# Matrixeigs/PowerSystemsReliabilityAssessment

Hardware: AMD Instinct MI355X
Metric: Monte Carlo DC-OPF scenarios/sec (RTS-24 HL2 non-sequential) (higher is better)
Workload: dtype f64

## Files before the change

### powersystemsreliabilityassessment_amd/csrc/relmc_core.hip

```cpp
#include <hip/hip_runtime.h>

#include <cmath>
#include <cstddef>
#include <cstdio>
#include <cstdlib>
#include <cstring>
#include <memory>
#include <new>
#include <type_traits>

#include "relmc_ctx.h"
#ifdef RELMC_DEV_SWITCHES
#include "relmc_dev_switches.h"
#endif
#include "relmc_kernels.hip"

static_assert(sizeof(relmc::DevAcc) == sizeof(relmc_acc), "device accumulator image must match relmc_acc");

namespace relmc_host {

const char* const kNoCtx = "relmc: null context";

int fail(relmc_ctx* ctx, int code, const std::string& msg)
{
// ... 9 lines not shown
    a.feastol = o.feastol; a.gradtol = o.gradtol; a.comptol = o.comptol; a.costtol = o.costtol;
    a.xi = o.xi; a.sigma = o.sigma; a.z0 = o.z0; a.alpha_min = o.alpha_min; a.max_stepsize = o.max_stepsize;
    a.fail_threshold = 1e-4;
    return a;
}

namespace {
template <class TL>
int grid_for(relmc_ctx* ctx, int64_t n)
{
    const int64_t groups = ((n + TL::SPW - 1) / TL::SPW + TL::WPB - 1) / TL::WPB;
    int64_t g = (int64_t)ctx->num_cu * ctx->blocks_per_cu;
    if (g > groups) g = groups;
    if (g < 1) g = 1;
    return (int)g;
}

template <int MODE, class TL>
int launch_eval_t(relmc_ctx* ctx, EvalArgs& a, int* rows_out, hipEvent_t ev_start, hipEvent_t ev_stop, int alt)
{
    int blocks = grid_for<TL>(ctx, a.n);
    if (MODE == 6) {
        if (blocks > 64) blocks = 64;
        const size_t n = 2 * (size_t)ctx->nb, stride = n * (n + 1), need = stride * (size_t)blocks * TL::WPB * TL::SPW;
        HIP_TRY(ctx, ctx->retry.dense.grow(need));
        a.dense = ctx->retry.dense.get(); a.dense_stride = stride;
    }
    HIP_TRY(ctx, ctx->dpartial.grow(sizeof(PartialT<TL>) * 64 * TL::WPB * (size_t)blocks));
    a.partial = ctx->dpartial.get();
    a.scen_doubles = alt ? ctx->alt_scen_doubles[alt - 1] : ctx->scen_doubles;
    a.prio_mode = blocks != ctx->num_cu * ctx->blocks_per_cu ? 0u : (ctx->blocks_per_cu == 2 ? 1u : (ctx->blocks_per_cu == 1 && TL::WPB >= 8 ? 2u : 0u));
    a.stash_off = alt ? ctx->alt_stash_off[alt - 1] : ctx->stash_off;
    a.case_bytes = (uint32_t)offsetof(DevCaseT<TL>, task);
#if defined(RELMC_PHASE_TIMING) || defined(RELMC_TRACE)
    HIP_TRY(ctx, ctx->dtiming.grow(8 * 65536));
    a.timing = ctx->dtiming.get(); ctx->timing_waves = blocks * TL::WPB;
#else
    a.timing = nullptr;
#endif
    a.tail_groups = 0;
    if constexpr (MODE == 0 && std::is_same<TL, Tile24>::value) {
        a.tail_rec = nullptr; a.tail_count = nullptr;
        const TailPlan plan(a.n, (int64_t)blocks * TL::WPB);
        if (plan.T > 0 && !ctx->sw.static_tail) {
            { const int rc = fail_count_ensure(ctx); if (rc) return rc; }
            HIP_TRY(ctx, ctx->dtail.grow(sizeof(TailRecT<TL>) * (size_t)plan.items()));
            a.tail_groups = plan.T; a.tail_rec = ctx->dtail.get(); a.tail_count = ctx->retry.fail_count.get() + 1;
        }
        ctx->last_tail_groups = a.tail_groups; ctx->tail_launches += a.tail_groups > 0;
        if (verbose()) fprintf(stderr, "relmc: fused launch of %lld scenarios on %d wavefronts: tail groups T = %d%s\n", (long long)a.n, blocks * TL::WPB, a.tail_groups,
                               a.tail_groups ? "" : (ctx->sw.static_tail ? " (static_tail)" : " (fewer than 2 T groups per wavefront)"));
    }
    HIP_TRY(ctx, hipEventRecord(ev_start ? ev_start : ctx->ev0, ctx->stream));
    bool launched = false;
    if constexpr (MODE == 0 && std::is_same<TL, Tile24>::value) {
        if (alt == 0 && ctx->shape_static && !ctx->sw.dynamic_shape) {
            hipLaunchKernelGGL((relmc_eval_kernel<0, Tile24, ShapeRts24>), dim3(blocks), dim3(64 * Tile24::WPB), ctx->lds_bytes, ctx->stream,
                               reinterpret_cast<const DevCaseT<Tile24>*>(ctx->dcase.get()), a);
            launched = true;
        }
    }
    if (!launched)
        hipLaunchKernelGGL((relmc_eval_kernel<MODE, TL>), dim3(blocks), dim3(64 * TL::WPB), alt ? ctx->alt_lds_bytes[alt - 1] : ctx->lds_bytes, ctx->stream,
                           reinterpret_cast<const DevCaseT<TL>*>(alt ? ctx->dcase_alt[alt - 1].get() : ctx->dcase.get()), a);
    HIP_TRY(ctx, hipGetLastError());
    if constexpr (MODE == 0 && std::is_same<TL, Tile24>::value) {
// ... 417 lines not shown
```

### powersystemsreliabilityassessment_amd/csrc/relmc_ctx.h

```cpp
#pragma once
#include <hip/hip_runtime.h>

#include <cmath>
#include <cstdint>
#include <functional>
#include <memory>
#include <string>
#include <type_traits>
#include <vector>

#include "../../include/relmc.h"
#include "relmc_dev.h"

struct relmc_switches {
    bool no_retry = false;
    bool retry_dense_first = false;
    bool nsq_no_stretch = false;
    bool db_no_probe = false;
    bool dynamic_shape = false;
    bool static_tail = false;
};

namespace relmc_host {
template <class T, bool Pinned = false>
class Buffer {
public:
    Buffer() = default;
    Buffer(Buffer&& o) noexcept : p_(o.p_), n_(o.n_) { o.p_ = nullptr; o.n_ = 0; }
    Buffer& operator=(Buffer&& o) noexcept
    {
        if (this != &o) { reset(); p_ = o.p_; n_ = o.n_; o.p_ = nullptr; o.n_ = 0; }
        return *this;
    }
    ~Buffer() { reset(); }
    T* get() const { return p_; }
    size_t size() const { return n_; }
    void reset()
    {
        if (p_) (void)(Pinned ? hipHostFree(p_) : hipFree(p_));
        p_ = nullptr; n_ = 0;
    }
    hipError_t grow(size_t n)
    {
        if (n <= n_) return hipSuccess;
        reset();
        void* p = nullptr;
        const hipError_t e = Pinned ? hipHostMalloc(&p, sizeof(T) * n, hipHostMallocDefault) : hipMalloc(&p, sizeof(T) * n);
        if (e == hipSuccess) { p_ = static_cast<T*>(p); n_ = n; }
        return e;
    }
private:
    T* p_ = nullptr;
    size_t n_ = 0;
// ... 298 lines not shown
```

### powersystemsreliabilityassessment_amd/csrc/relmc_debug.hip

```cpp
#include <cstdio>
#include <cstring>
#include <memory>

#include "relmc_ctx.h"
#include "relmc_shape_rts24.h"

using namespace relmc_host;

extern "C" {

int32_t relmc_debug_schedule(const relmc_ctx* ctx, int32_t* out9)
{
    if (!ctx || !out9 || !ctx->has_case) return RELMC_ERR_INVALID;
    auto fill = [&](const auto& C) {
        int ntask = 0;
        for (int p = 0; p < C.npass; ++p) ntask += C.pass_ntask[p];
        out9[0] = C.npass_upd; out9[1] = C.npass_inv; out9[2] = C.npass - C.npass_upd - C.npass_inv; out9[3] = C.noff;
        out9[4] = C.nzero; out9[5] = (int)C.nws; out9[6] = (int)ctx->lds_bytes; out9[7] = ctx->blocks_per_cu; out9[8] = ntask;
        if (verbose()) fprintf(stderr, "relmc: modelled LDS conflict cycles per Newton step %ld -> %ld\n", ctx->conflict_before, ctx->conflict_after);
        if (verbose()) fprintf(stderr, "relmc: longest line / injection list per bus slot: %d %d / %d %d\n", (int)C.maxdeg_s[0], (int)C.maxdeg_s[1], (int)C.maxinj_s[0], (int)C.maxinj_s[1]);
        if (verbose()) { fprintf(stderr, "relmc: tasks per pass:"); for (int p = 0; p < C.npass; ++p) fprintf(stderr, " %d", (int)C.pass_ntask[p]); fprintf(stderr, "\n"); }
    };
    if (ctx->tile == 0) fill(ctx->hcase24); else fill(ctx->hcase96);
    return RELMC_OK;
// ... 10 lines not shown
    std::vector<uint32_t> keys((size_t)n * ow, 0u);
    for (int64_t r = 0; r < n; ++r) for (int k = 0; k < ncomp; ++k) if (states_host[(size_t)r * ncomp + k]) keys[(size_t)r * ow + (k >> 5)] |= 1u << (k & 31);
    DevBuf<uint32_t> dk; DevBuf<double> dd, dn; DevBuf<int32_t> dm;
    if (dk.grow(keys.size()) != hipSuccess || dd.grow((size_t)n) != hipSuccess || dm.grow((size_t)n) != hipSuccess || dn.grow((size_t)n * nb) != hipSuccess)
        return fail(ctx, RELMC_ERR_HIP, "dense simulation: device allocation failed");
    int rc = RELMC_OK;
    if (hipMemcpy(dk.get(), keys.data(), sizeof(uint32_t) * keys.size(), hipMemcpyHostToDevice) != hipSuccess) rc = fail(ctx, RELMC_ERR_HIP, "dense simulation: H2D failed");
    EvalArgs a = make_args(o);
    a.n = n; a.memo_keys = dk.get(); a.db_first = 0; a.dns = dd.get(); a.status = dm.get(); a.nodal = dn.get();
    int rows = 0;
    if (rc == RELMC_OK) rc = launch_eval(ctx, 6, a, &rows);
    if (rc == RELMC_OK) rc = finish_timing(ctx);
    std::vector<int32_t> meta((size_t)n);
    if (rc == RELMC_OK && (hipMemcpy(dns_host, dd.get(), sizeof(double) * (size_t)n, hipMemcpyDeviceToHost) != hipSuccess ||
                           hipMemcpy(meta.data(), dm.get(), sizeof(int32_t) * (size_t)n, hipMemcpyDeviceToHost) != hipSuccess ||
                           (nodal_host && hipMemcpy(nodal_host, dn.get(), sizeof(double) * (size_t)n * nb, hipMemcpyDeviceToHost) != hipSuccess)))
        rc = fail(ctx, RELMC_ERR_HIP, "dense simulation: D2H failed");
    if (rc) return rc;
    for (int64_t r = 0; r < n; ++r) { if (status_host) status_host[r] = meta[(size_t)r] & 3; if (iters_host) iters_host[r] = (int32_t)((uint32_t)meta[(size_t)r] >> 8); }
    return RELMC_OK;
}

int32_t relmc_debug_phase_cycles(relmc_ctx* ctx, unsigned long long* out8)
{
    if (!ctx || !out8) return RELMC_ERR_INVALID;
    for (int k = 0; k < 8; ++k) out8[k] = 0;
    if (!ctx->dtiming.get() || ctx->timing_waves <= 0) return RELMC_OK;
    std::vector<unsigned long long> h((size_t)ctx->timing_waves * 8);
    HIP_TRY(ctx, hipMemcpy(h.data(), ctx->dtiming.get(), h.size() * sizeof(unsigned long long), hipMemcpyDeviceToHost));
    for (int w = 0; w < ctx->timing_waves; ++w) for (int k = 0; k < 8; ++k) out8[k] += h[(size_t)w * 8 + k];
    return RELMC_OK;
}

int32_t relmc_debug_trace(relmc_ctx* ctx, double* out, int32_t n_doubles)
{
    if (!ctx || !out || n_doubles < 0) return RELMC_ERR_INVALID;
    for (int k = 0; k < n_doubles; ++k) out[k] = 0.0;
    if (!ctx->dtiming.get() || n_doubles > 8 * 65536) return RELMC_OK;
    HIP_TRY(ctx, hipMemcpy(out, ctx->dtiming.get(), sizeof(double) * n_doubles, hipMemcpyDeviceToHost));
    return RELMC_OK;
}

int32_t relmc_debug_shape(const relmc_case_desc* d, const int32_t* order_hint, int32_t n_hint, int32_t* case_out, int32_t* static_out)
{
    if (static_out) ShapeRts24::values(static_out);
    if (case_out) {
        if (!d) return RELMC_ERR_INVALID;
        SymOpts so = sym_opts_default();
        if (order_hint && n_hint > 0) { so.order_hint = order_hint; so.n_hint = n_hint; }
        std::string err;
        SymGeom g;
        const int rc = with_symbolic(d, 0, so, g, err, [&](const auto& C) { shape_of(C, g.stash_off, g.scen_doubles, case_out); return (int)RELMC_OK; });
        if (rc) return rc < 0 ? rc : -rc;
    }
    return SF_COUNT;
}

int64_t relmc_debug_stretch_len(int64_t batch, int64_t done, double beta, double beta_limit, int64_t round, int32_t* final_out)
{
    if (batch <= 0 || batch > kStretchMaxBatch || done < 0 || round < 0) return RELMC_ERR_INVALID;
    const Stretch s = stretch_length(batch, done, beta, beta_limit, stretch_per(batch), round);
    if (final_out) *final_out = s.final ? 1 : 0;
    return s.len;
}

int32_t relmc_debug_shape_path(const relmc_ctx* ctx)
{
    if (!ctx || !ctx->has_case) return RELMC_ERR_INVALID;
    return ctx->shape_static && !ctx->sw.dynamic_shape ? 1 : 0;
}

int32_t relmc_debug_tail_plan(int64_t n, int32_t waves, int64_t* a_begin, int64_t* a_end, int32_t* owner, int64_t* group)
{
    if (n < 0 || waves <= 0) return RELMC_ERR_INVALID;
    const TailPlan plan(n, waves);
    for (int64_t w = 0; w < waves; ++w) { if (a_begin) a_begin[w] = plan.begin(w); if (a_end) a_end[w] = plan.cut(w); }
    for (int64_t p = 0; p < plan.items(); ++p) { if (owner) owner[p] = (int32_t)plan.owner(p); if (group) group[p] = plan.group(p); }
    return plan.T;
}

int32_t relmc_debug_tail_groups(const relmc_ctx* ctx, int64_t* launches_out, int32_t* waves_out)
{
    if (!ctx) return RELMC_ERR_INVALID;
    if (launches_out) *launches_out = ctx->tail_launches;
    if (waves_out) *waves_out = ctx->has_case && ctx->tile == 0 ? ctx->num_cu * ctx->blocks_per_cu * Tile24::WPB : 0;
    return ctx->last_tail_groups;
}

int32_t relmc_debug_set(relmc_ctx* ctx, const char* key, int32_t value)
{
    if (!ctx || !key) return RELMC_ERR_INVALID;
    const bool v = value != 0;
    if (!std::strcmp(key, "no_retry")) ctx->sw.no_retry = v;
    else if (!std::strcmp(key, "retry_dense_first")) ctx->sw.retry_dense_first = v;
    else if (!std::strcmp(key, "nsq_no_stretch")) ctx->sw.nsq_no_stretch = v;
    else if (!std::strcmp(key, "db_no_probe")) ctx->sw.db_no_probe = v;
    else if (!std::strcmp(key, "dynamic_shape")) ctx->sw.dynamic_shape = v;
    else if (!std::strcmp(key, "static_tail")) ctx->sw.static_tail = v;
    else return fail(ctx, RELMC_ERR_INVALID, std::string("relmc_debug_set: unknown switch ") + key);
    return RELMC_OK;
}

}
```

### powersystemsreliabilityassessment_amd/csrc/relmc_dev.h

```cpp
#pragma once
#include <stdint.h>

namespace relmc {

template <int RW_, int BS_, int LS_, int IS_, int NCOMPMAX_, int MAXPASS_, int MAXOFF_, int WPB_>
struct TileT {
    static constexpr int RW = RW_;
    static constexpr int BS = BS_;
    static constexpr int LS = LS_;
    static constexpr int IS = IS_;
    static constexpr int NBT = BS_ * RW_;
    static constexpr int NLT = LS_ * RW_;
    static constexpr int NIT = IS_ * RW_;
    static constexpr int SPW = 64 / RW_;
    static constexpr int NCOMPMAX = NCOMPMAX_;
    static constexpr int OW = NCOMPMAX_ / 32;
    static constexpr int MAXPASS = MAXPASS_;
    static constexpr int MAXOFF = MAXOFF_;
    static constexpr int WPB = WPB_;
    static_assert(BS_ <= 2 && LS_ <= 3 && IS_ <= 4, "the per-lane flag word has room for 2 bus, 3 line and 4 injection slots");
};
using Tile24 = TileT<16, 2, 3, 4, 128, 96, 160, 4>;
using Tile96 = TileT<64, 2, 2, 3, 256, 64, 320, 8>;
constexpr int DEGMAX = 8;
// ... 70 lines not shown
    int64_t n;
    int32_t policy, max_it;
    double feastol, gradtol, comptol, costtol, xi, sigma, z0, alpha_min, max_stepsize;
    const uint8_t* states;
    double* dns;
    double* nodal;
    int32_t* status;
    int32_t* iters;
    void* partial;
    uint32_t prio_mode;
    uint32_t scen_doubles;
    uint32_t stash_off;
    uint32_t case_bytes;
    unsigned long long* timing;
    double fail_threshold;
    const double* load_scale;
    const uint32_t* seq_masks;
    const uint32_t* seq_offsets;
    const uint16_t* seq_hours;
    const double* load_factors;
    double* curt;
    int32_t seq_nyears, seq_hpy;
    const uint32_t* memo_keys;
    const uint32_t* memo_perm;
    const uint32_t* memo_start;
    int64_t db_first;
    uint32_t* fail_count;
    FailRec* fail_list;
    uint32_t fail_cap;
    int32_t tail_groups;
    int64_t unit_base;
    union { double* dense; void* tail_rec; };
    union { uint64_t dense_stride; uint32_t* tail_count; };
};

struct ScreenTab {
    int32_t nl, ng, valid, pad;
    double total_load;
    double sum_pmin, sum_rng;
    const double* pmin;
    const double* rng;
    const double* f_min;
    const double* f_rng;
    const double* f_load;
    const double* lim;
    const double* gpair;
    const double* hmat;
    const uint8_t* bridge;
};

struct DevAcc {
    long long n, n_fail, n_singular, n_infeasible, n_nonconverged, sum_iters;
    long long comp_fail[256];
    long long n_screened;
    double sum_dns, sum_dns2;
    double sum_nodal[128];
};

constexpr int FIN_ITEMS = 8 + 256 + 128;

constexpr int NCOMPMAX = 128;
constexpr int SEQ_NCOMPMAX = 256;
struct SeqCase {
    int32_t ncomp, hpy, mw, pad;
    double mttf[SEQ_NCOMPMAX], mttr[SEQ_NCOMPMAX];
};
// ... 78 lines not shown
```

### powersystemsreliabilityassessment_amd/csrc/relmc_dev_switches.h

```cpp
#pragma once
#include <cstdlib>

#include "relmc_ctx.h"

inline void relmc_dev_switches_context(relmc_switches& sw)
{
    sw.no_retry = std::getenv("RELMC_NO_RETRY") != nullptr; sw.retry_dense_first = std::getenv("RELMC_RETRY_DENSE_FIRST") != nullptr;
    sw.nsq_no_stretch = std::getenv("RELMC_NSQ_NO_STRETCH") != nullptr; sw.db_no_probe = std::getenv("RELMC_DB_NO_PROBE") != nullptr;
}

inline void relmc_dev_switches_schedule(relmc_host::SymOpts& so)
{
    if (const char* q = std::getenv("RELMC_PLACE_WW")) so.place_ww = std::atol(q);
    if (const char* q = std::getenv("RELMC_PLACE_MOVES")) so.place_moves = std::atoi(q);
    so.no_quarter = std::getenv("RELMC_NO_QUARTER") != nullptr; so.no_half = std::getenv("RELMC_NO_HALF") != nullptr;
    if (const char* q = std::getenv("RELMC_SCEN_PAD4")) so.scen_pad4 = std::atoi(q);
    so.no_bwd_half = std::getenv("RELMC_NO_BWD_HALF") != nullptr; so.no_bus_map = std::getenv("RELMC_NO_BUS_MAP") != nullptr;
}
```

### powersystemsreliabilityassessment_amd/csrc/relmc_kernels.hip

```cpp
#include "relmc_devfn.h"
#include "relmc_shape_rts24.h"

namespace relmc {


constexpr int kPrioBit = 12;
constexpr int kMinWaves = 2;
#define DINF __builtin_inf()
#define RELOAD_FENCE() __asm__ volatile("" ::: "memory")
#define SLOT_FENCE() __builtin_amdgcn_sched_barrier(0)
#ifdef RELMC_PASS_NOUNROLL
#define PASS_LOOP _Pragma("nounroll")
#else
#define PASS_LOOP
#endif
constexpr int kPfMask = 0xc0;
constexpr int kPfMaskWide = 0xc6;
#define PFSITE(k) (((PF_MASK >> (k)) & 1) != 0)
constexpr int kShadowMask = 0xff;
constexpr int kShadowMaskWide = 0xff;
#define PASS_IDLE(d) (((d).x & 0xffffu) == ((d).y >> 16))
#define PASS_IDLE_INV(d) ((d).y != 0u)
#ifdef RELMC_PHASE_TIMING
#define PT_DECL unsigned long long pt_[8] = {0, 0, 0, 0, 0, 0, 0, 0}; unsigned long long pt0_ = __builtin_readcyclecounter();
#define PT_MARK(k) { const unsigned long long n_ = __builtin_readcyclecounter(); pt_[k] += n_ - pt0_; pt0_ = n_; }
#define PT_FLUSH if (a.timing && lane == 0) { for (int k = 0; k < 8; ++k) a.timing[((size_t)blockIdx.x * WPB + (tid >> 6)) * 8 + k] = pt_[k]; }
#else
#define PT_DECL
#define PT_MARK(k)
#define PT_FLUSH
#endif
#if defined(RELMC_PHASE_TIMING) && defined(RELMC_PT_INIT)
#undef PT_MARK
#define PT_MARK(k) { const unsigned long long n_ = __builtin_readcyclecounter(); pt_[(k) == 7 ? 7 : 6] += n_ - pt0_; pt0_ = n_; }
#define PT_IMARK(k) { const unsigned long long n_ = __builtin_readcyclecounter(); pt_[k] += n_ - pt0_; pt0_ = n_; }
#else
#define PT_IMARK(k)
#endif

template <int MODE_, class TL, class SH = ShapeDynamic>
__global__ void __launch_bounds__(64 * TL::WPB, kMinWaves) relmc_eval_kernel(const DevCaseT<TL>* __restrict__ gcase, const EvalArgs a)
{
    constexpr int MODE = MODE_ == 5 ? 0 : (MODE_ == 6 ? 4 : MODE_);
    constexpr bool DENSE = MODE_ == 6;
    constexpr int PAIR_MASK = TL::RW == 16 ? kRpairMask : kRpairMaskWide;
#define PAIRSITE(k) (((PAIR_MASK >> (k)) & 1) != 0)
    constexpr int PF_MASK = TL::RW == 16 ? kPfMask : kPfMaskWide;
    constexpr bool SHADOW = (((TL::RW == 16 ? kShadowMask : kShadowMaskWide) >> MODE) & 1) != 0;
    constexpr int RW = TL::RW, BS = TL::BS, LS = TL::LS, IS = TL::IS, NBT = TL::NBT, WPB = TL::WPB, SPW = TL::SPW, OW = TL::OW;
    using DevCase = DevCaseT<TL>;
    using Partial = PartialT<TL>;
    extern __shared__ __attribute__((aligned(16))) unsigned char smem[];
    constexpr uint32_t OPT_BYTES = 128;
    double* const OPT = reinterpret_cast<double*>(smem);
#define A_(k, name) OPT[k]
    DevCase& C = *reinterpret_cast<DevCase*>(smem + OPT_BYTES);
    const DevCase& TASKSRC = *gcase;
    const DevCase& TABL = C;
    const DevCase& TABI = (RW == 64) ? *gcase : C;
    const DevCase& TABG = (RW == 64) ? *gcase : C;
    const int tid = threadIdx.x, lane = tid & 63, rlane = lane & (RW - 1), row = tid / RW;
    const uint32_t case_bytes = a.case_bytes;
    {
        const uint32_t* src = reinterpret_cast<const uint32_t*>(gcase);
        uint32_t* dst = reinterpret_cast<uint32_t*>(smem + OPT_BYTES);
        if (tid == 0) { OPT[0] = a.feastol; OPT[1] = a.gradtol; OPT[2] = a.comptol; OPT[3] = a.costtol; OPT[4] = a.xi; OPT[5] = a.sigma;
                        OPT[6] = a.z0; OPT[7] = a.alpha_min; OPT[8] = a.max_stepsize; OPT[9] = a.fail_threshold; }
        for (uint32_t i = tid; i < case_bytes / 4; i += 64 * WPB) dst[i] = src[i];
    }
    __syncthreads();
    double* const W = reinterpret_cast<double*>(smem + OPT_BYTES + ((case_bytes + 15u) & ~15u)) + (size_t)row * SHAPE(scen_doubles, a.scen_doubles);
    const int nlp = SHAPE(nl, C.nl), nip = SHAPE(ninj, C.ninj);
    double* const LR = W;
    double* const IR = W + 4 * (nlp + 1);
    const int maxdeg0 = SHAPE(maxdeg0, C.maxdeg_s[0]), maxdeg1 = SHAPE(maxdeg1, C.maxdeg_s[1]), maxinj0 = SHAPE(maxinj0, C.maxinj_s[0]), maxinj1 = SHAPE(maxinj1, C.maxinj_s[1]);
    double* const Stash = W + SHAPE(stash_off, a.stash_off) + 2 * rlane;
    const double* const StashJ = W + SHAPE(stash_off, a.stash_off);
    double* const Lam = W + SHAPE(stash_off, a.stash_off) + 2 * IS * RW + 2;
    uint32_t* const OB = reinterpret_cast<uint32_t*>(Lam + NBT);

    const int ng = SHAPE(ng, C.ng), ncomp = C.ncomp, nb = SHAPE(nb, C.nb);
// ... 116 lines not shown
        }
        RELOAD_FENCE();
        win_valid = n_valid;
        win_groups = (int)((n_valid + 3u) >> 2);
        if (run < win_groups) win_groups = run;
    }
    PT_IMARK(0)
    for (int wg = wg0; wg < win_groups; ++wg) {
        const int64_t grp = WINDOWED ? wb + wg : wb;
        const int64_t sidx = grp * SPW + lane / RW;
        const bool live = WINDOWED ? (uint32_t)(wg * 4 + lane / RW) < win_valid : sidx < a.n;
        double lscale = 1.0;
        uint32_t wgt = 1;
        int seq_year = 0, seq_hour = 0;
        RELOAD_FENCE();

        uint32_t sf = 0;
#define L_ON(s) (((sf >> (s)) & 1u) != 0)
#define L_ACT(s) (((sf >> (3 + (s))) & 1u) != 0)
#define I_ON(s) (((sf >> (6 + (s))) & 1u) != 0)
#define I_BOX(s) (((sf >> (10 + (s))) & 1u) != 0)
#define B_PIN(t) (((sf >> (14 + (t))) & 1u) != 0)
#define B_DROP(t) (((sf >> (16 + (t))) & 1u) != 0)
#define L_PIN(s) (((sf >> (18 + (s))) & 1u) != 0)
#define L_C1Z(s) (((sf >> (21 + (s))) & 1u) != 0)
#define L_C2Z(s) (((sf >> (24 + (s))) & 1u) != 0)
        double LFv[LS], LGv[LS], lzp[LS], lzm[LS], lmup[LS], lmum[LS], cBv[LS];
        double ip[IS], izp[IS], izm[IS], imup[IS], imum[IS];
        double bth[BS], bla[BS], cBd[BS];
        double gamma = 1.0, fval = 0.0, f0 = 0.0, alphap = 1.0, alphad = 1.0, zmu = 0.0;
        uint32_t niq = 0;
        int it = 0, status = 0;
        bool infeas = false, singular = false, iterating = false;
        uint32_t lozero = 0;
#define ISC(s) ((RW * (s) + rlane >= ng) ? lscale : 1.0)
#define ILOV(s, lo_) (((lozero >> (s)) & 1u) ? 0.0 : (lo_) * ISC(s))
#pragma unroll
        for (int s = 0; s < LS; ++s) { LFv[s] = 0; LGv[s] = 0; lzp[s] = 1; lzm[s] = 1; lmup[s] = 1; lmum[s] = 1; cBv[s] = 0; }
#pragma unroll
        for (int s = 0; s < IS; ++s) { ip[s] = 0; izp[s] = 1; izm[s] = 1; imup[s] = 1; imum[s] = 1; }
#pragma unroll
        for (int t = 0; t < BS; ++t) { bth[t] = 0; bla[t] = 0; cBd[t] = 0; }

        if (live) {
            if (MODE == 2) {
                int lo_ = 0, hi_ = a.seq_nyears;
                while (hi_ - lo_ > 1) { const int mid = (lo_ + hi_) >> 1; if ((int64_t)a.seq_offsets[mid] <= sidx) lo_ = mid; else hi_ = mid; }
                seq_year = lo_;
                seq_hour = a.seq_hours[(size_t)seq_year * a.seq_hpy + (size_t)(sidx - a.seq_offsets[seq_year])];
                const uint32_t* m = a.seq_masks + ((size_t)seq_year * a.seq_hpy + seq_hour) * OW;
                if (rlane < OW) OB[rlane] = m[rlane];
                lscale = a.load_factors[seq_hour];
            } else if (MODE == 3) {
                const uint32_t s0 = a.memo_start[sidx];
                wgt = a.memo_start[sidx + 1] - s0;
                if (rlane < OW) OB[rlane] = a.memo_keys[(size_t)a.memo_perm[s0] * OW + rlane];
            } else if (MODE == 4) {
                if (rlane < OW) OB[rlane] = a.memo_keys[(size_t)(a.db_first + (a.memo_perm ? (int64_t)a.memo_perm[sidx] : sidx)) * OW + rlane];
                if (a.load_scale) lscale = a.load_scale[sidx];
            } else if (MODE == 7) {
                if (rlane < OW) OB[rlane] = a.memo_keys[(size_t)a.memo_perm[sidx] * OW + rlane];
            } else {
                if (rlane < OW) OB[rlane] = 0u;
                RELOAD_FENCE();
                if (WINDOWED) {
                    if (rlane < OW) OB[rlane] = WIN[4 * (wg * 4 + lane / RW) + rlane];
// ... 307 lines not shown
                        double mu = z0v; if (z0_small) { if (1.0 / z > z0v) mu = 1.0 / z; }
                        izp[s] = z; izm[s] = z; imup[s] = mu; imum[s] = mu;
                        nq += 2;
                    }
                    fl += C.i_tab[RW * s + rlane][2] * ip[s];
                }
            }
#pragma unroll
            for (int t = 0; t < BS; ++t) if (vb[t] < nb) Lam[vb[t]] = 0.0;
            if (rlane == 0) st2(W + SHAPE(stash_off, a.stash_off) + 2 * IS * RW, 0.0, 0.0);
            niq = row_add<RW>(nq);
            fval = row_sum<RW>(fl);
            f0 = fval;
            iterating = !singular;
            status = singular ? 3 : 0;
        }

        PT_IMARK(5)
        PT_MARK(0)
        while (__any(iterating)) {
            if (prio_first) {
                if ((__builtin_readcyclecounter() >> kPrioBit) & 1ull) __builtin_amdgcn_s_setprio(3); else __builtin_amdgcn_s_setprio(0);
            }
            RELOAD_FENCE();
            if constexpr (RW == 16) {
                __asm__ volatile("" : "+v"(sf));
#pragma unroll
                for (int s = 0; s < LS; ++s) __asm__ volatile("" : "+v"(linfo[s]));
#pragma unroll
                for (int s = 0; s < IS; ++s) __asm__ volatile("" : "+v"(iinfo[s]));
#pragma unroll
                for (int t = 0; t < BS; ++t) __asm__ volatile("" : "+v"(vb[t]));
            }
            if (iterating) {
                double mx_gh = -DINF, mx_x = 0.0, mx_z = 0.0, mx_lx = 0.0, mx_lammu = 0.0;
                bool nanx = false;
                double gown[LS];
#pragma unroll
                for (int s = 0; s < LS; ++s) {
                    const int l = RW * s + rlane;
                    double g = 0.0, q = 0.0;
                    double lx = LGv[s];
                    if (L_ACT(s)) {
                        const double b = lb(s), rr = lr(s);
                        const double hp = LFv[s] - rr, hm = -LFv[s] - rr;
                        double rzp, rzm; frcp_pair<PAIRSITE(0)>(lzp[s], lzm[s], rzp, rzm);
                        g = b * b * (lmup[s] * rzp + lmum[s] * rzm);
                        lx = __builtin_fma(b, lmup[s] - lmum[s], lx);
                        q = b * ((lmup[s] * hp + gamma) * rzp - (lmum[s] * hm + gamma) * rzm);
                        mx_gh = vmax(mx_gh, vmax(hp, hm));
                        mx_z = vmax(mx_z, vmax(lzp[s], lzm[s]));
                        mx_lammu = vmax(mx_lammu, vmax(lmup[s], lmum[s]));
                    }
                    gown[s] = g;
                    if (l < nlp) { st2(LR + 4 * l, g, lx); st2(LR + 4 * l + 2, lx + q, LFv[s]); }
                    SLOT_FENCE();
                }
#pragma unroll
                for (int s = 0; s < IS; ++s) {
                    const int j = RW * s + rlane;
                    double invD = 0.0, npd = 0.0;
                    const double pv = ip[s];
                    mx_x = vmax(mx_x, __builtin_fabs(pv));
                    nanx = nanx || pv != pv;
                    if (I_BOX(s)) {
                        const d2 hl = IHL(s, j);
                        const double hp = pv - hl.x, hm = ILOV(s, hl.y) - pv;
                        const double lxp = ICOST(s, j) - Lam[iinfo[s] & 0xff] + (imup[s] - imum[s]);
                        if constexpr ((RW == 16 && kInjNform) || (RW == 64 && kInjNformWide)) {
                            const double N = __builtin_fma(imup[s], izm[s], imum[s] * izp[s]);
                            const double rN = frcp(N), zz = izp[s] * izm[s];
                            invD = zz * rN;
                            npd = __builtin_fma(lxp, zz, (imup[s] * hp + gamma) * izm[s] - (imum[s] * hm + gamma) * izp[s]) * rN;
                        } else {
                        double rzp, rzm; frcp_pair<PAIRSITE(1)>(izp[s], izm[s], rzp, rzm);
                        const double D = imup[s] * rzp + imum[s] * rzm;
                        const double np = lxp + (imup[s] * hp + gamma) * rzp - (imum[s] * hm + gamma) * rzm;
                        invD = frcp(D); npd = np * invD;
                        }
                        mx_lx = vmax(mx_lx, __builtin_fabs(lxp));
                        mx_gh = vmax(mx_gh, vmax(hp, hm));
                        mx_z = vmax(mx_z, vmax(izp[s], izm[s]));
                        mx_lammu = vmax(mx_lammu, vmax(imup[s], imum[s]));
                    }
                    if (j < nip) IR[j] = pv;
                    st2(Stash + 2 * RW * s, invD, npd);
                    SLOT_FENCE();
                }
                PT_MARK(1)
                if (rlane == 0) { st2(LR + 4 * nlp, 0.0, 0.0); st2(LR + 4 * nlp + 2, 0.0, 0.0); IR[nip] = 0.0; }
                uint32_t lblk_pf[LS]; uint32_t zo_pf = 0;
                if constexpr (PFSITE(1)) {
#pragma unroll
                    for (int s = 0; s < LS; ++s) lblk_pf[s] = C.l_blk[RW * s + rlane];
                    zo_pf = C.zero_off[rlane];
                }
                unsigned long long pl_pf[BS], pj_pf[BS];
                if constexpr (PFSITE(2)) {
#pragma unroll
                    for (int t = 0; t < BS; ++t) { const int bq = vb[t] < nb ? vb[t] : 0; pl_pf[t] = PLIST(t, bq); pj_pf[t] = JLIST(t, bq); }
                }
                double vown[LS];
                {
                    double gp[LS];
#pragma unroll
                    for (int s = 0; s < LS; ++s) gp[s] = LR[4 * (lpart[s] >= 0 ? lpart[s] : nlp)];
#pragma unroll
                    for (int s = 0; s < LS; ++s) vown[s] = (((linfo[s] >> 24) & LF_OWNER) && !L_PIN(s)) ? -(gown[s] + gp[s]) : 0.0;
                }
                double d00[BS], d11[BS], r0[BS], r1[BS];
#pragma unroll
                for (int t = 0; t < BS; ++t) {
                    const int bi = vb[t];
                    d00[t] = 0; d11[t] = 0; r0[t] = 0; r1[t] = 0;
                    if (bi < nb) {
                        double md = 0.0, lx = 0.0, nq_ = 0.0, bal = 0.0, E = 0.0, ssum = 0.0;
                        const unsigned long long pl = PFSITE(2) ? pl_pf[t] : PLIST(t, bi), pj = PFSITE(2) ? pj_pf[t] : JLIST(t, bi);
#pragma unroll
                        for (int e = 0; e < DEGMAX; e += 2) {
                            if (e >= (t == 0 ? maxdeg0 : maxdeg1)) break;
                            const uint32_t ent0 = (uint32_t)(pl >> (8 * e)) & 0xffu, ent1 = (uint32_t)(pl >> (8 * e + 8)) & 0xffu;
                            const int l0 = (int)(ent0 & 0x7f), l1 = (int)(ent1 & 0x7f);
                            const double sg0 = (ent0 & 0x80) ? -1.0 : 1.0, sg1 = (ent1 & 0x80) ? -1.0 : 1.0;
                            const d2 ra0 = ld2(LR + 4 * l0), rb0 = ld2(LR + 4 * l0 + 2), ra1 = ld2(LR + 4 * l1), rb1 = ld2(LR + 4 * l1 + 2);
                            md += ra0.x;
                            lx = __builtin_fma(sg0, ra0.y, lx);
                            nq_ = __builtin_fma(sg0, rb0.x, nq_);
                            bal = __builtin_fma(sg0, rb0.y, bal);
                            md += ra1.x;
                            lx = __builtin_fma(sg1, ra1.y, lx);
                            nq_ = __builtin_fma(sg1, rb1.x, nq_);
                            bal = __builtin_fma(sg1, rb1.y, bal);
                        }
#pragma unroll
                        for (int e = 0; e < BINJMAX; e += 2) {
                            if (e >= (t == 0 ? maxinj0 : maxinj1)) break;
                            const int j0 = (int)((uint32_t)(pj >> (8 * e)) & 0xffu), j1 = (int)((uint32_t)(pj >> (8 * e + 8)) & 0xffu);
                            const d2 sh0 = ld2(StashJ + 2 * j0), sh1 = ld2(StashJ + 2 * j1);
                            const double p0 = IR[j0], p1 = IR[j1];
                            bal -= p0; E += sh0.x; ssum += sh0.y;
                            bal -= p1; E += sh1.x; ssum += sh1.y;
                        }
                        if (B_PIN(t)) {
                            d00[t] = 1.0; r0[t] = 0.0;
                            mx_lammu = vmax(mx_lammu, __builtin_fabs(lx));
                        } else {
                            d00[t] = md; r0[t] = -nq_;
                            mx_lx = vmax(mx_lx, __builtin_fabs(lx));
                        }
                        if (B_DROP(t)) {
                            d11[t] = -1.0; r1[t] = 0.0;
                        } else {
                            d11[t] = -E; r1[t] = -bal - ssum;
                            mx_gh = vmax(mx_gh, __builtin_fabs(bal));
                            mx_lammu = vmax(mx_lammu, __builtin_fabs(bla[t]));
                        }
                        mx_x = vmax(mx_x, __builtin_fabs(bth[t]));
                        nanx = nanx || bth[t] != bth[t];
                    }
                }
                RELOAD_FENCE();
                if constexpr (DENSE) {
                    const int n = 2 * nb, n1 = n + 1;
                    volatile double* A = a.dense + ((size_t)blockIdx.x * (WPB * SPW) + (size_t)(tid / RW)) * (size_t)a.dense_stride;
                    for (int e = rlane; e < n * n1; e += RW) A[e] = 0.0;
                    __threadfence_block();
#pragma unroll
                    for (int s = 0; s < LS; ++s) {
                        if ((linfo[s] >> 24) & LF_OWNER) {
                            const int f = linfo[s] & 0xff, t = (linfo[s] >> 8) & 0xff;
                            const int hi = f < t ? t : f, lo = f < t ? f : t;
                            const double c1 = L_C1Z(s) ? 0.0 : cBv[s], c2 = L_C2Z(s) ? 0.0 : cBv[s];
                            A[(2 * hi) * n1 + 2 * lo] = vown[s]; A[(2 * lo) * n1 + 2 * hi] = vown[s];
                            A[(2 * hi) * n1 + 2 * lo + 1] = c1; A[(2 * lo + 1) * n1 + 2 * hi] = c1;
                            A[(2 * hi + 1) * n1 + 2 * lo] = c2; A[(2 * lo) * n1 + 2 * hi + 1] = c2;
                        }
                    }
#pragma unroll
                    for (int t = 0; t < BS; ++t) {
                        const int bi = vb[t];
                        if (bi < nb) {
                            A[(2 * bi) * n1 + 2 * bi] = d00[t]; A[(2 * bi) * n1 + 2 * bi + 1] = cBd[t];
                            A[(2 * bi + 1) * n1 + 2 * bi] = cBd[t]; A[(2 * bi + 1) * n1 + 2 * bi + 1] = d11[t];
                            A[(2 * bi) * n1 + n] = r0[t]; A[(2 * bi + 1) * n1 + n] = r1[t];
                        }
                    }
                    __threadfence_block();
                } else {
#pragma unroll
                for (int s = 0; s < LS; ++s) {
                    if ((linfo[s] >> 24) & LF_OWNER) {
                        const double c1 = L_C1Z(s) ? 0.0 : cBv[s];
                        const double c2 = L_C2Z(s) ? 0.0 : cBv[s];
                        double* blk = W + (PFSITE(1) ? lblk_pf[s] : (uint32_t)C.l_blk[RW * s + rlane]);
                        st2(blk, vown[s], c1); st2(blk + 2, c2, 0.0);
                    }
                }
                if constexpr (PFSITE(1)) {
                    for (int z = rlane; z < nzero; z += RW) {
                        const uint32_t zn = C.zero_off[z + RW < TL::MAXOFF ? z + RW : z];
                        double* blk = W + zo_pf; st2(blk, 0.0, 0.0); st2(blk + 2, 0.0, 0.0);
                        zo_pf = zn;
                    }
                } else
                for (int z = rlane; z < nzero; z += RW) { double* blk = W + C.zero_off[z]; st2(blk, 0.0, 0.0); st2(blk + 2, 0.0, 0.0); }
#pragma unroll
                for (int t = 0; t < BS; ++t) {
                    const int bi = vb[t];
                    if (bi < nb) {
                        st2(W + 4 * bi, d00[t], cBd[t]); st2(W + 4 * bi + 2, cBd[t], d11[t]);
                        st2(W + off_rhs + 2 * bi, r0[t], r1[t]);
                    }
                }
                }

                PT_MARK(2)
                double o_ct = 0.0, o_cc = 0.0, o_am = 0.0;
                if constexpr (PFSITE(7)) { o_ct = A_(2, comptol); o_cc = A_(3, costtol); o_am = A_(7, alpha_min); }
                mx_x = row_max<RW>(mx_x);
                const bool xnan = row_any<RW>(nanx, lane);
                if constexpr (!PFSITE(7)) { o_ct = A_(2, comptol); o_cc = A_(3, costtol); }
                bool conv = it > 0 && zmu < o_ct * (1.0 + mx_x) && __builtin_fabs(fval - f0) < o_cc * (1.0 + __builtin_fabs(f0));
#ifdef RELMC_TRACE
                {
                    const double t_gh = row_max<RW>(mx_gh), t_z = row_max<RW>(mx_z), t_lx = row_max<RW>(mx_lx), t_lm = row_max<RW>(mx_lammu);
                    if (a.timing && blockIdx.x == 0 && tid == 0 && it < 60) {
                        double* o = reinterpret_cast<double*>(a.timing) + 8 * it;
                        o[0] = t_gh / (1.0 + vmax(mx_x, t_z)); o[1] = t_lx / (1.0 + t_lm); o[2] = zmu / (1.0 + mx_x);
                        o[3] = __builtin_fabs(fval - f0) / (1.0 + __builtin_fabs(f0)); o[4] = alphap; o[5] = alphad; o[6] = gamma; o[7] = fval;
                    }
                }
#endif
                if (__any(conv)) {
                    mx_gh = row_max<RW>(mx_gh); mx_z = row_max<RW>(mx_z); mx_lx = row_max<RW>(mx_lx); mx_lammu = row_max<RW>(mx_lammu);
                    conv = conv && mx_gh < A_(0, feastol) * (1.0 + vmax(mx_x, mx_z)) && mx_lx < A_(1, gradtol) * (1.0 + mx_lammu);
                }
                if (conv) { status = 0; iterating = false; }
                else if (it > 0 && (xnan || alphap < (PFSITE(7) ? o_am : A_(7, alpha_min)) || alphad < (PFSITE(7) ? o_am : A_(7, alpha_min)) || gamma < eps || gamma > 1.0 / eps)) { status = 2; iterating = false; }
                else if (it >= a.max_it) { status = 1; iterating = false; }
            }
            PT_MARK(3)
            RELOAD_FENCE();
            if (iterating) {
                f0 = fval;
                it += 1;
                if constexpr (DENSE) {
                    const int n = 2 * nb, n1 = n + 1;
                    volatile double* A = a.dense + ((size_t)blockIdx.x * (WPB * SPW) + (size_t)(tid / RW)) * (size_t)a.dense_stride;
                    double* const Fm = W;
                    bool singular_k = false;
                    for (int k = 0; k < n; ++k) {
                        double best = -1.0; int bi = n;
                        for (int i = k + rlane; i < n; i += RW) { const double v = __builtin_fabs(A[(size_t)i * n1 + k]); if (v > best) { best = v; bi = i; } }
                        const double mx = row_max<RW>(best);
                        const uint32_t cand = (best == mx) ? (uint32_t)bi : (uint32_t)n;
                        const int p = (int)row_min_u32<RW>(cand);
                        if (!(mx > 0.0)) { singular_k = true; break; }
                        if (p != k) for (int j = k + rlane; j <= n; j += RW) { const double u = A[(size_t)k * n1 + j], v = A[(size_t)p * n1 + j]; A[(size_t)k * n1 + j] = v; A[(size_t)p * n1 + j] = u; }
                        __threadfence_block();
                        const double rp = 1.0 / A[(size_t)k * n1 + k];
                        for (int i = k + 1 + rlane; i < n; i += RW) Fm[i] = A[(size_t)i * n1 + k] * rp;
                        RELOAD_FENCE();
                        for (int i = k + 1; i < n; ++i) {
                            const double f = Fm[i];
                            if (f != 0.0) for (int j = k + 1 + rlane; j <= n; j += RW) A[(size_t)i * n1 + j] = A[(size_t)i * n1 + j] - f * A[(size_t)k * n1 + j];
                        }
                        __threadfence_block();
                    }
                    for (int k = n - 1; k >= 0 && !singular_k; --k) {
                        double sdot = 0.0;
                        for (int j = k + 1 + rlane; j < n; j += RW) sdot = __builtin_fma(A[(size_t)k * n1 + j], Fm[j], sdot);
                        sdot = row_sum<RW>(sdot);
// ... 202 lines not shown
                            const d2 hl = IHL(s, j);
                            const double hp = ip[s] - hl.x, hm = ILOV(s, hl.y) - ip[s];
                            const double dzp = -hp - izp[s] - dpv[s], dzm = -hm - izm[s] + dpv[s];
                            double rzp, rzm; frcp_pair<PAIRSITE(4)>(izp[s], izm[s], rzp, rzm);
                            const double dmup = -imup[s] + (gamma - imup[s] * dzp) * rzp;
                            const double dmum = -imum[s] + (gamma - imum[s] * dzm) * rzm;
                            tp = vmax(tp, vmax(-dzp * rzp, -dzm * rzm));
                            double rmp, rmm; frcp1_pair<PAIRSITE(5)>(imup[s], imum[s], rmp, rmm);
                            td = vmax(td, vmax(-dmup * rmp, -dmum * rmm));
                            step2 = __builtin_fma(dpv[s], dpv[s], step2);
                        }
                    }
                    SLOT_FENCE();
                }
                step2 = row_sum<RW>(step2);
#ifdef RELMC_TRACE
                if (a.timing && blockIdx.x == 0 && tid < RW && it < 40) {
                    double* o2 = reinterpret_cast<double*>(a.timing) + 512 + 512 * it;
                    for (int t = 0; t < BS; ++t) if (vb[t] < nb) { o2[vb[t]] = dth[t]; o2[128 + vb[t]] = dla[t]; }
                    for (int s = 0; s < IS; ++s) o2[256 + RW * s + rlane] = dpv[s];
                    if (it == 1) for (int t = 0; t < BS; ++t) if (vb[t] < nb) (reinterpret_cast<double*>(a.timing) + 512 + 512 * 40)[vb[t]] = (double)C.b_ext[vb[t]];
                }
#endif
                if (!(PFSITE(6) ? step2 <= o_ms * o_ms : step2 <= A_(8, max_stepsize) * A_(8, max_stepsize))) {
                    status = 2; iterating = false;
                } else {
                    double o_xi = 0.0, o_sg = 0.0;
                    if constexpr (PFSITE(6)) { o_xi = A_(4, xi); o_sg = A_(5, sigma); }
                    tp = row_max<RW>(tp); td = row_max<RW>(td);
                    if constexpr (!PFSITE(6)) o_xi = A_(4, xi);
                    alphap = tp > 0.0 ? vmin(o_xi * frcp(tp), 1.0) : 1.0;
                    alphad = td > 0.0 ? vmin(o_xi * frcp(td), 1.0) : 1.0;
                    double zl = 0.0, fl = 0.0;
#pragma unroll
                    for (int s = 0; s < LS; ++s) {
                        if (L_ACT(s)) {
                            const double hp = LFv[s] - lr(s), hm = -LFv[s] - lr(s);
                            const double dzp = -hp - lzp[s] - dF[s], dzm = -hm - lzm[s] + dF[s];
                            double rzp, rzm; frcp_pair<PAIRSITE(6)>(lzp[s], lzm[s], rzp, rzm);
                            const double dmup = -lmup[s] + (gamma - lmup[s] * dzp) * rzp;
                            const double dmum = -lmum[s] + (gamma - lmum[s] * dzm) * rzm;
                            lzp[s] = __builtin_fma(alphap, dzp, lzp[s]); lzm[s] = __builtin_fma(alphap, dzm, lzm[s]);
                            lmup[s] = __builtin_fma(alphad, dmup, lmup[s]); lmum[s] = __builtin_fma(alphad, dmum, lmum[s]);
                            zl = __builtin_fma(lzp[s], lmup[s], zl); zl = __builtin_fma(lzm[s], lmum[s], zl);
                        }
                        LFv[s] = __builtin_fma(alphap, dF[s], LFv[s]);
                        LGv[s] = __builtin_fma(alphad, dG[s], LGv[s]);
                        SLOT_FENCE();
                    }
#pragma unroll
                    for (int s = 0; s < IS; ++s) {
                        if (I_BOX(s)) {
                            const int j = RW * s + rlane;
                            const d2 hl = IHL(s, j);
                            const double hp = ip[s] - hl.x, hm = ILOV(s, hl.y) - ip[s];
                            const double dzp = -hp - izp[s] - dpv[s], dzm = -hm - izm[s] + dpv[s];
                            double rzp, rzm; frcp_pair<PAIRSITE(7)>(izp[s], izm[s], rzp, rzm);
                            const double dmup = -imup[s] + (gamma - imup[s] * dzp) * rzp;
                            const double dmum = -imum[s] + (gamma - imum[s] * dzm) * rzm;
                            ip[s] = __builtin_fma(alphap, dpv[s], ip[s]);
                            izp[s] = __builtin_fma(alphap, dzp, izp[s]); izm[s] = __builtin_fma(alphap, dzm, izm[s]);
                            imup[s] = __builtin_fma(alphad, dmup, imup[s]); imum[s] = __builtin_fma(alphad, dmum, imum[s]);
                            zl = __builtin_fma(izp[s], imup[s], zl); zl = __builtin_fma(izm[s], imum[s], zl);
                        }
                        fl = __builtin_fma(ICOST(s, RW * s + rlane), ip[s], fl);
                        SLOT_FENCE();
                    }
#pragma unroll
                    for (int t = 0; t < BS; ++t) {
                        bth[t] = __builtin_fma(alphap, dth[t], bth[t]); bla[t] = __builtin_fma(alphad, dla[t], bla[t]);
                        if (vb[t] < nb) Lam[vb[t]] = bla[t];
                    }
                    zmu = row_sum<RW>(zl);
                    fval = row_sum<RW>(fl);
                    if (niq > 0) gamma = (PFSITE(6) ? o_sg : A_(5, sigma)) * zmu / (double)niq;
                }
                PT_MARK(6)
            }
        }

        PT_MARK(6)
        using TailRec = TailRecT<TL>;
        RELOAD_FENCE();
        const int tp = WINDOWED ? *TP : -1;
        const bool park = WINDOWED && tp >= 0;
        uint32_t tflag = 0;
        if (live) {
            double dns = fval + C.total_load * lscale;
            if (dns < 0.1) dns = 0.0;
            const bool fail = dns > a.fail_threshold;
            bool defer = false;
            if (a.fail_list && (status == 1 || status == 2)) {
                uint32_t pos = 0;
                if (rlane == 0) pos = atomicAdd(a.fail_count, 1u);
                pos = __shfl(pos, lane & ~(RW - 1));
                if (pos < a.fail_cap) {
                    defer = true;
                    FailRec* fr = a.fail_list + pos;
                    if (rlane < OW) fr->mask[rlane] = OB[rlane];
                    if (rlane == 0) {
                        const int64_t u = (MODE == 0 && WINDOWED) ? wb * 4 + WINL[wg * 4 + lane / RW]
                                          : (MODE == 2 ? (int64_t)seq_year * a.seq_hpy + seq_hour
                                          : (MODE == 7 ? (int64_t)a.memo_perm[sidx]
                                          : (MODE == 4 && a.memo_perm ? (int64_t)a.memo_perm[sidx] : sidx)));
                        fr->unit = (unsigned long long)(u + a.unit_base); fr->weight = wgt; fr->pad = 0;
                    }
                }
            }
// ... 195 lines not shown
```

Baseline: 61.99 million.

## Skip convergence norm reductions unless cheap stage-1 test passes

Splits the interior-point convergence check into two stages. The x-norm, NaN flag and the complementarity/cost test are now computed at the end of the step update. The expensive per-slot max tracking of residual norms in the front half is compiled out, via a template specialisation, for wavefronts where no row passes stage 1. This removes many vmax operations and cross-lane reductions per Newton iteration in the common non-converged case, at the cost of code duplication (two instantiations of the front half), extra register pressure and a wave-uniform branch. It also adds a debug switch and trip counters.

Measured after the change: 63.30 million (median of 6 runs). 1.02x the previous value.

```diff
diff --git a/powersystemsreliabilityassessment_amd/csrc/relmc_core.hip b/powersystemsreliabilityassessment_amd/csrc/relmc_core.hip
--- a/powersystemsreliabilityassessment_amd/csrc/relmc_core.hip
+++ b/powersystemsreliabilityassessment_amd/csrc/relmc_core.hip
@@ -65,6 +65,7 @@
     a.prio_mode = blocks != ctx->num_cu * ctx->blocks_per_cu ? 0u : (ctx->blocks_per_cu == 2 ? 1u : (ctx->blocks_per_cu == 1 && TL::WPB >= 8 ? 2u : 0u));
     a.stash_off = alt ? ctx->alt_stash_off[alt - 1] : ctx->stash_off;
     a.case_bytes = (uint32_t)offsetof(DevCaseT<TL>, task);
+    a.norms_always = ctx->sw.norms_always ? 1u : 0u;
 #if defined(RELMC_PHASE_TIMING) || defined(RELMC_TRACE)
     HIP_TRY(ctx, ctx->dtiming.grow(8 * 65536));
     a.timing = ctx->dtiming.get(); ctx->timing_waves = blocks * TL::WPB;
diff --git a/powersystemsreliabilityassessment_amd/csrc/relmc_ctx.h b/powersystemsreliabilityassessment_amd/csrc/relmc_ctx.h
--- a/powersystemsreliabilityassessment_amd/csrc/relmc_ctx.h
+++ b/powersystemsreliabilityassessment_amd/csrc/relmc_ctx.h
@@ -19,6 +19,7 @@
     bool db_no_probe = false;
     bool dynamic_shape = false;
     bool static_tail = false;
+    bool norms_always = false;
 };
 
 namespace relmc_host {
diff --git a/powersystemsreliabilityassessment_amd/csrc/relmc_debug.hip b/powersystemsreliabilityassessment_amd/csrc/relmc_debug.hip
--- a/powersystemsreliabilityassessment_amd/csrc/relmc_debug.hip
+++ b/powersystemsreliabilityassessment_amd/csrc/relmc_debug.hip
@@ -66,6 +66,17 @@
     return RELMC_OK;
 }
 
+int32_t relmc_debug_norm_trips(relmc_ctx* ctx, unsigned long long* out2)
+{
+    if (!ctx || !out2) return RELMC_ERR_INVALID;
+    out2[0] = out2[1] = 0;
+    if (!ctx->dtiming.get() || ctx->timing_waves <= 0) return RELMC_OK;
+    std::vector<unsigned long long> h((size_t)ctx->timing_waves * 2);
+    HIP_TRY(ctx, hipMemcpy(h.data(), ctx->dtiming.get() + (size_t)ctx->timing_waves * 8, h.size() * sizeof(unsigned long long), hipMemcpyDeviceToHost));
+    for (int w = 0; w < ctx->timing_waves; ++w) for (int k = 0; k < 2; ++k) out2[k] += h[(size_t)w * 2 + k];
+    return RELMC_OK;
+}
+
 int32_t relmc_debug_trace(relmc_ctx* ctx, double* out, int32_t n_doubles)
 {
     if (!ctx || !out || n_doubles < 0) return RELMC_ERR_INVALID;
@@ -131,6 +142,7 @@
     else if (!std::strcmp(key, "db_no_probe")) ctx->sw.db_no_probe = v;
     else if (!std::strcmp(key, "dynamic_shape")) ctx->sw.dynamic_shape = v;
     else if (!std::strcmp(key, "static_tail")) ctx->sw.static_tail = v;
+    else if (!std::strcmp(key, "norms_always")) ctx->sw.norms_always = v;
     else return fail(ctx, RELMC_ERR_INVALID, std::string("relmc_debug_set: unknown switch ") + key);
     return RELMC_OK;
 }
diff --git a/powersystemsreliabilityassessment_amd/csrc/relmc_dev.h b/powersystemsreliabilityassessment_amd/csrc/relmc_dev.h
--- a/powersystemsreliabilityassessment_amd/csrc/relmc_dev.h
+++ b/powersystemsreliabilityassessment_amd/csrc/relmc_dev.h
@@ -126,6 +126,7 @@
     int64_t unit_base;
     union { double* dense; void* tail_rec; };
     union { uint64_t dense_stride; uint32_t* tail_count; };
+    uint32_t norms_always;
 };
 
 struct ScreenTab {
diff --git a/powersystemsreliabilityassessment_amd/csrc/relmc_dev_switches.h b/powersystemsreliabilityassessment_amd/csrc/relmc_dev_switches.h
--- a/powersystemsreliabilityassessment_amd/csrc/relmc_dev_switches.h
+++ b/powersystemsreliabilityassessment_amd/csrc/relmc_dev_switches.h
@@ -7,6 +7,7 @@
 {
     sw.no_retry = std::getenv("RELMC_NO_RETRY") != nullptr; sw.retry_dense_first = std::getenv("RELMC_RETRY_DENSE_FIRST") != nullptr;
     sw.nsq_no_stretch = std::getenv("RELMC_NSQ_NO_STRETCH") != nullptr; sw.db_no_probe = std::getenv("RELMC_DB_NO_PROBE") != nullptr;
+    sw.norms_always = std::getenv("RELMC_NORMS_ALWAYS") != nullptr;
 }
 
 inline void relmc_dev_switches_schedule(relmc_host::SymOpts& so)
diff --git a/powersystemsreliabilityassessment_amd/csrc/relmc_kernels.hip b/powersystemsreliabilityassessment_amd/csrc/relmc_kernels.hip
--- a/powersystemsreliabilityassessment_amd/csrc/relmc_kernels.hip
+++ b/powersystemsreliabilityassessment_amd/csrc/relmc_kernels.hip
@@ -19,15 +19,20 @@
 #define PFSITE(k) (((PF_MASK >> (k)) & 1) != 0)
 constexpr int kShadowMask = 0xff;
 constexpr int kShadowMaskWide = 0xff;
+constexpr int kNormSplitMask = 0xff;
+constexpr int kNormSplitMaskWide = 0;
 #define PASS_IDLE(d) (((d).x & 0xffffu) == ((d).y >> 16))
 #define PASS_IDLE_INV(d) ((d).y != 0u)
 #ifdef RELMC_PHASE_TIMING
-#define PT_DECL unsigned long long pt_[8] = {0, 0, 0, 0, 0, 0, 0, 0}; unsigned long long pt0_ = __builtin_readcyclecounter();
+#define PT_DECL unsigned long long pt_[8] = {0, 0, 0, 0, 0, 0, 0, 0}, ptn_[2] = {0, 0}; unsigned long long pt0_ = __builtin_readcyclecounter();
 #define PT_MARK(k) { const unsigned long long n_ = __builtin_readcyclecounter(); pt_[k] += n_ - pt0_; pt0_ = n_; }
-#define PT_FLUSH if (a.timing && lane == 0) { for (int k = 0; k < 8; ++k) a.timing[((size_t)blockIdx.x * WPB + (tid >> 6)) * 8 + k] = pt_[k]; }
+#define PT_TRIP(k) ptn_[k] += 1;
+#define PT_FLUSH if (a.timing && lane == 0) { for (int k = 0; k < 8; ++k) a.timing[((size_t)blockIdx.x * WPB + (tid >> 6)) * 8 + k] = pt_[k]; \
+                                              for (int k = 0; k < 2; ++k) a.timing[(size_t)gridDim.x * WPB * 8 + ((size_t)blockIdx.x * WPB + (tid >> 6)) * 2 + k] = ptn_[k]; }
 #else
 #define PT_DECL
 #define PT_MARK(k)
+#define PT_TRIP(k)
 #define PT_FLUSH
 #endif
 #if defined(RELMC_PHASE_TIMING) && defined(RELMC_PT_INIT)
@@ -47,6 +52,7 @@
 #define PAIRSITE(k) (((PAIR_MASK >> (k)) & 1) != 0)
     constexpr int PF_MASK = TL::RW == 16 ? kPfMask : kPfMaskWide;
     constexpr bool SHADOW = (((TL::RW == 16 ? kShadowMask : kShadowMaskWide) >> MODE) & 1) != 0;
+    constexpr bool NSPLIT = (((TL::RW == 16 ? kNormSplitMask : kNormSplitMaskWide) >> MODE) & 1) != 0;
     constexpr int RW = TL::RW, BS = TL::BS, LS = TL::LS, IS = TL::IS, NBT = TL::NBT, WPB = TL::WPB, SPW = TL::SPW, OW = TL::OW;
     using DevCase = DevCaseT<TL>;
     using Partial = PartialT<TL>;
@@ -229,6 +235,8 @@
         uint32_t niq = 0;
         int it = 0, status = 0;
         bool infeas = false, singular = false, iterating = false;
+        double x_inf = 0.0;
+        bool x_nan = false, stage1 = false;
         uint32_t lozero = 0;
 #define ISC(s) ((RW * (s) + rlane >= ng) ? lscale : 1.0)
 #define ILOV(s, lo_) (((lozero >> (s)) & 1u) ? 0.0 : (lo_) * ISC(s))
@@ -602,7 +610,14 @@
 #pragma unroll
                 for (int t = 0; t < BS; ++t) __asm__ volatile("" : "+v"(vb[t]));
             }
-            if (iterating) {
+#ifdef RELMC_TRACE
+            const bool need_norms = true;
+#else
+            const bool need_norms = !NSPLIT || __builtin_amdgcn_readfirstlane((int)(__any(iterating && stage1) != 0 || a.norms_always != 0)) != 0;
+#endif
+            PT_TRIP(need_norms ? 1 : 0)
+            auto front_half = [&](auto norms_c) __attribute__((always_inline)) {
+                constexpr bool NORMS = decltype(norms_c)::value;
                 double mx_gh = -DINF, mx_x = 0.0, mx_z = 0.0, mx_lx = 0.0, mx_lammu = 0.0;
                 bool nanx = false;
                 double gown[LS];
@@ -618,9 +633,11 @@
                         g = b * b * (lmup[s] * rzp + lmum[s] * rzm);
                         lx = __builtin_fma(b, lmup[s] - lmum[s], lx);
                         q = b * ((lmup[s] * hp + gamma) * rzp - (lmum[s] * hm + gamma) * rzm);
-                        mx_gh = vmax(mx_gh, vmax(hp, hm));
-                        mx_z = vmax(mx_z, vmax(lzp[s], lzm[s]));
-                        mx_lammu = vmax(mx_lammu, vmax(lmup[s], lmum[s]));
+                        if constexpr (NORMS) {
+                            mx_gh = vmax(mx_gh, vmax(hp, hm));
+                            mx_z = vmax(mx_z, vmax(lzp[s], lzm[s]));
+                            mx_lammu = vmax(mx_lammu, vmax(lmup[s], lmum[s]));
+                        }
                     }
                     gown[s] = g;
                     if (l < nlp) { st2(LR + 4 * l, g, lx); st2(LR + 4 * l + 2, lx + q, LFv[s]); }
@@ -631,8 +648,7 @@
                     const int j = RW * s + rlane;
                     double invD = 0.0, npd = 0.0;
                     const double pv = ip[s];
-                    mx_x = vmax(mx_x, __builtin_fabs(pv));
-                    nanx = nanx || pv != pv;
+                    if constexpr (!NSPLIT) { mx_x = vmax(mx_x, __builtin_fabs(pv)); nanx = nanx || pv != pv; }
                     if (I_BOX(s)) {
                         const d2 hl = IHL(s, j);
                         const double hp = pv - hl.x, hm = ILOV(s, hl.y) - pv;
@@ -648,10 +664,12 @@
                         const double np = lxp + (imup[s] * hp + gamma) * rzp - (imum[s] * hm + gamma) * rzm;
                         invD = frcp(D); npd = np * invD;
                         }
-                        mx_lx = vmax(mx_lx, __builtin_fabs(lxp));
-                        mx_gh = vmax(mx_gh, vmax(hp, hm));
-                        mx_z = vmax(mx_z, vmax(izp[s], izm[s]));
-                        mx_lammu = vmax(mx_lammu, vmax(imup[s], imum[s]));
+                        if constexpr (NORMS) {
+                            mx_lx = vmax(mx_lx, __builtin_fabs(lxp));
+                            mx_gh = vmax(mx_gh, vmax(hp, hm));
+                            mx_z = vmax(mx_z, vmax(izp[s], izm[s]));
+                            mx_lammu = vmax(mx_lammu, vmax(imup[s], imum[s]));
+                        }
                     }
                     if (j < nip) IR[j] = pv;
                     st2(Stash + 2 * RW * s, invD, npd);
@@ -713,22 +731,25 @@
                         }
                         if (B_PIN(t)) {
                             d00[t] = 1.0; r0[t] = 0.0;
-                            mx_lammu = vmax(mx_lammu, __builtin_fabs(lx));
+                            if constexpr (NORMS) mx_lammu = vmax(mx_lammu, __builtin_fabs(lx));
                         } else {
                             d00[t] = md; r0[t] = -nq_;
-                            mx_lx = vmax(mx_lx, __builtin_fabs(lx));
+                            if constexpr (NORMS) mx_lx = vmax(mx_lx, __builtin_fabs(lx));
                         }
                         if (B_DROP(t)) {
                             d11[t] = -1.0; r1[t] = 0.0;
                         } else {
                             d11[t] = -E; r1[t] = -bal - ssum;
-                            mx_gh = vmax(mx_gh, __builtin_fabs(bal));
-                            mx_lammu = vmax(mx_lammu, __builtin_fabs(bla[t]));
-                        }
-                        mx_x = vmax(mx_x, __builtin_fabs(bth[t]));
-                        nanx = nanx || bth[t] != bth[t];
-                    }
-                }
+                            if constexpr (NORMS) {
+                                mx_gh = vmax(mx_gh, __builtin_fabs(bal));
+                                mx_lammu = vmax(mx_lammu, __builtin_fabs(bla[t]));
+                            }
+                        }
+                        if constexpr (!NSPLIT) { mx_x = vmax(mx_x, __builtin_fabs(bth[t])); nanx = nanx || bth[t] != bth[t]; }
+                    }
+                }
+                double o_ct = 0.0, o_cc = 0.0, o_am = 0.0;
+                if constexpr (NSPLIT && PFSITE(7)) o_am = A_(7, alpha_min);
                 RELOAD_FENCE();
                 if constexpr (DENSE) {
                     const int n = 2 * nb, n1 = n + 1;
@@ -785,12 +806,17 @@
                 }
 
                 PT_MARK(2)
-                double o_ct = 0.0, o_cc = 0.0, o_am = 0.0;
-                if constexpr (PFSITE(7)) { o_ct = A_(2, comptol); o_cc = A_(3, costtol); o_am = A_(7, alpha_min); }
-                mx_x = row_max<RW>(mx_x);
-                const bool xnan = row_any<RW>(nanx, lane);
-                if constexpr (!PFSITE(7)) { o_ct = A_(2, comptol); o_cc = A_(3, costtol); }
-                bool conv = it > 0 && zmu < o_ct * (1.0 + mx_x) && __builtin_fabs(fval - f0) < o_cc * (1.0 + __builtin_fabs(f0));
+                bool conv = false, xnan = false;
+                if constexpr (NSPLIT) {
+                    mx_x = x_inf; xnan = x_nan;
+                    conv = NORMS && stage1;
+                } else {
+                    if constexpr (PFSITE(7)) { o_ct = A_(2, comptol); o_cc = A_(3, costtol); o_am = A_(7, alpha_min); }
+                    mx_x = row_max<RW>(mx_x);
+                    xnan = row_any<RW>(nanx, lane);
+                    if constexpr (!PFSITE(7)) { o_ct = A_(2, comptol); o_cc = A_(3, costtol); }
+                    conv = it > 0 && zmu < o_ct * (1.0 + mx_x) && __builtin_fabs(fval - f0) < o_cc * (1.0 + __builtin_fabs(f0));
+                }
 #ifdef RELMC_TRACE
                 {
                     const double t_gh = row_max<RW>(mx_gh), t_z = row_max<RW>(mx_z), t_lx = row_max<RW>(mx_lx), t_lm = row_max<RW>(mx_lammu);
@@ -801,13 +827,16 @@
                     }
                 }
 #endif
-                if (__any(conv)) {
+                if constexpr (NORMS) if (__any(conv)) {
                     mx_gh = row_max<RW>(mx_gh); mx_z = row_max<RW>(mx_z); mx_lx = row_max<RW>(mx_lx); mx_lammu = row_max<RW>(mx_lammu);
                     conv = conv && mx_gh < A_(0, feastol) * (1.0 + vmax(mx_x, mx_z)) && mx_lx < A_(1, gradtol) * (1.0 + mx_lammu);
                 }
                 if (conv) { status = 0; iterating = false; }
                 else if (it > 0 && (xnan || alphap < (PFSITE(7) ? o_am : A_(7, alpha_min)) || alphad < (PFSITE(7) ? o_am : A_(7, alpha_min)) || gamma < eps || gamma > 1.0 / eps)) { status = 2; iterating = false; }
                 else if (it >= a.max_it) { status = 1; iterating = false; }
+            };
+            if (iterating) {
+                if (need_norms) front_half(std::true_type{}); else front_half(std::false_type{});
             }
             PT_MARK(3)
             RELOAD_FENCE();
@@ -1076,6 +1105,7 @@
                     alphap = tp > 0.0 ? vmin(o_xi * frcp(tp), 1.0) : 1.0;
                     alphad = td > 0.0 ? vmin(o_xi * frcp(td), 1.0) : 1.0;
                     double zl = 0.0, fl = 0.0;
+                    double xm = 0.0; bool xn = false;
 #pragma unroll
                     for (int s = 0; s < LS; ++s) {
                         if (L_ACT(s)) {
@@ -1108,16 +1138,26 @@
                             zl = __builtin_fma(izp[s], imup[s], zl); zl = __builtin_fma(izm[s], imum[s], zl);
                         }
                         fl = __builtin_fma(ICOST(s, RW * s + rlane), ip[s], fl);
+                        if constexpr (NSPLIT) { xm = vmax(xm, __builtin_fabs(ip[s])); xn = xn || ip[s] != ip[s]; }
                         SLOT_FENCE();
                     }
+                    double o_ct = 0.0, o_cc = 0.0;
+                    if constexpr (NSPLIT) { o_ct = A_(2, comptol); o_cc = A_(3, costtol); }
 #pragma unroll
                     for (int t = 0; t < BS; ++t) {
                         bth[t] = __builtin_fma(alphap, dth[t], bth[t]); bla[t] = __builtin_fma(alphad, dla[t], bla[t]);
-                        if (vb[t] < nb) Lam[vb[t]] = bla[t];
+                        if (vb[t] < nb) {
+                            Lam[vb[t]] = bla[t];
+                            if constexpr (NSPLIT) { xm = vmax(xm, __builtin_fabs(bth[t])); xn = xn || bth[t] != bth[t]; }
+                        }
                     }
                     zmu = row_sum<RW>(zl);
                     fval = row_sum<RW>(fl);
                     if (niq > 0) gamma = (PFSITE(6) ? o_sg : A_(5, sigma)) * zmu / (double)niq;
+                    if constexpr (NSPLIT) {
+                        x_inf = row_max<RW>(xm); x_nan = row_any<RW>(xn, lane);
+                        stage1 = zmu < o_ct * (1.0 + x_inf) && __builtin_fabs(fval - f0) < o_cc * (1.0 + __builtin_fabs(f0));
+                    }
                 }
                 PT_MARK(6)
             }
```
